# yhw-yhw/TalkSHOW

Hardware: NVIDIA H100
Metric: smplx_motion_frames_per_sec (higher is better)
Workload: dtype f32

## Files before the change

talkshow_b200/csrc/api.cu:

```cuda
#include "convstack.h"
#include "pixelcnn.h"

using namespace ts;

static std::string g_create_err;

float* ts_engine::upload(const std::vector<float>& h) {
  if (host_only) return nullptr;
  void* d = dmalloc(h.size() * sizeof(float));
  TS_CUDA(cudaMemcpy(d, h.data(), h.size() * sizeof(float), cudaMemcpyHostToDevice));
  return (float*)d;
}
unsigned short* ts_engine::upload(const std::vector<unsigned short>& h) {
  if (host_only) return nullptr;
  void* d = dmalloc(h.size() * sizeof(unsigned short));
  TS_CUDA(cudaMemcpy(d, h.data(), h.size() * sizeof(unsigned short), cudaMemcpyHostToDevice));
  return (unsigned short*)d;
}
void* ts_engine::dmalloc(size_t bytes) {
  if (host_only) return nullptr;
  void* d = nullptr;
  TS_CUDA(cudaMalloc(&d, bytes ? bytes : 16));
  (alloc_sink ? *alloc_sink : owned).push_back(d);
  return d;
// ... 208 lines not shown
      TS_CUDA(cudaEventRecord(e->aux_fork, s));
      TS_CUDA(cudaStreamWaitEvent(e->aux_stream, e->aux_fork, 0));
    }
    for (int w = 0; w < 2; ++w) {
      cudaStream_t sw = (w == 1 && par) ? e->aux_stream : s;
      Act3 y = run_vq_decode(e, e->conv->vq[w], idx_c + (size_t)w * B * T, B, T, sw);
      act_to_btc(e, y, e->conv->vq[w].out_dim, poses, c0 + c1, w ? c0 : 0, sw);
    }
    if (par) {
      TS_CUDA(cudaEventRecord(e->aux_join, e->aux_stream));
      TS_CUDA(cudaStreamWaitEvent(s, e->aux_join, 0));
    }
  };
  e->ws.begin_sizing();
  body();
  size_t need = e->ws.need;
  e->ws.buf.ensure(need + 256);
  e->ws.begin(need);
  body();
  TS_API_END(e)
}
```

talkshow_b200/csrc/common.h:

```cpp
#pragma once
#include <cuda_runtime.h>
#include <stdint.h>

#include <cstdarg>
#include <cstdio>
#include <cstring>
#include <map>
#include <stdexcept>
#include <string>
#include <vector>

#include "../../include/talkshow_b200.h"

namespace ts {

struct Error : std::runtime_error {
  int code;
  Error(int c, const std::string& m) : std::runtime_error(m), code(c) {}
};

[[noreturn]] inline void fail(int code, const char* fmt, ...) {
  char buf[1024];
  va_list ap;
  va_start(ap, fmt);
// ... 47 lines not shown
    bytes = n;
  }
  void release() {
    if (p) cudaFree(p);
    p = nullptr;
    bytes = 0;
  }
  template <class T>
  T* as() const { return (T*)p; }
};

struct Workspace {
  DevBuf buf;
  size_t off = 0;
  size_t need = 0;
  bool sizing = false;
  void begin_sizing() { sizing = true; off = 0; need = 0; }
  void begin(size_t) { sizing = false; off = 0; }
  template <class T>
  T* alloc(size_t n) {
    size_t b = (n * sizeof(T) + 255) & ~size_t(255);
    size_t o = off;
    off += b;
    if (off > need) need = off;
    if (sizing) return nullptr;
    if (off > buf.bytes) fail(TS_ERR_CUDA, "workspace overflow (%zu > %zu)", off, buf.bytes);
    return (T*)((char*)buf.p + o);
  }
};

struct Layer {
  float* W = nullptr;
  float* W_hi = nullptr;
// ... 110 lines not shown
```

talkshow_b200/csrc/convstack.cu:

```cuda
#include "convstack.h"

#include <cmath>

namespace ts {

static const double BN_EPS = 1e-5;

struct Folded {
  std::vector<double> a, b;
};

static Folded bn_fold(const Ckpt& ck, const std::string& p, int c) {
  const float* g = ck.f32(p + "weight", {c});
  const float* be = ck.f32(p + "bias", {c});
  const float* mu = ck.f32(p + "running_mean", {c});
  const float* var = ck.f32(p + "running_var", {c});
  Folded f;
  f.a.resize(c);
  f.b.resize(c);
  for (int i = 0; i < c; ++i) {
    double a = (double)g[i] / std::sqrt((double)var[i] + BN_EPS);
    f.a[i] = a;
    f.b[i] = (double)be[i] - (double)mu[i] * a;
  }
// ... 186 lines not shown
  conv_auto(e, v.project, h, 1, 1, 0, y, h.T, ACT_NONE, nullptr, s);
  return y;
}

Act3 run_vq_decode(ts_engine* e, const VQNet& v, const int64_t* idx, int B, int T, cudaStream_t s) {
  Act3 q = new_act(e, B, T, 64, 0, s);
  gather_rows(e, v.codebook, 64, idx, q, s);
  return run_decoder(e, v, q, s);
}

}

using namespace ts;

template <class F>
static void run_sized(ts_engine* e, F&& body) {
  e->ws.begin_sizing();
  body();
  size_t need = e->ws.need;
  e->ws.buf.ensure(need + 256);
  e->ws.begin(need);
  body();
}

extern "C" int ts_latent_rows(int M) {
  int m = (M + 2 - 4) / 2 + 1;
  return (m + 2 - 4) / 2 + 1;
}

extern "C" int ts_load_audioenc(ts_engine* e, const ts_tensor* tensors, int n) {
  TS_API_BEGIN(e)
  Ckpt ck(tensors, n);
  if (!e->conv) e->conv = new ConvStacks();
  LoadScope scope(e, "audioenc");
  Trunk t;
  pack_trunk(e, ck, "", 64, 256, &t);
// ... 10 lines not shown
  if (!e->conv) e->conv = new ConvStacks();
  LoadScope scope(e, which ? "vq1" : "vq0");
  VQNet v;
  pack_vq(e, ck, &v);
  e->conv->vq[which] = v;
  scope.commit();
  TS_API_END(e)
}

extern "C" int ts_audio_encode(ts_engine* e, const float* mfcc, float* out, int B, int M, void* stream) {
  TS_API_BEGIN(e)
  ts::require_device(e);
  if (!e->conv || !e->conv->audio_loaded) fail(TS_ERR_NOT_LOADED, "audio encoder weights not loaded");
  if (B <= 0 || M < 4) fail(TS_ERR_INVALID, "ts_audio_encode: B=%d M=%d", B, M);
  cudaStream_t s = (cudaStream_t)stream;
  run_sized(e, [&] {
    Act3 x = new_act(e, B, M, 64, 1, s);
    nct_to_act(e, mfcc, 64, x, s);
    Act3 y = run_trunk(e, e->conv->audio, x, s);
    act_to_nct(e, y, 256, out, s);
  });
  TS_API_END(e)
}

extern "C" int ts_vq_decode(ts_engine* e, int which, const int64_t* idx, float* out, int B, int T, void* stream) {
  TS_API_BEGIN(e)
  ts::require_device(e);
  if (which < 0 || which > 1 || !e->conv || !e->conv->vq[which].loaded) fail(TS_ERR_NOT_LOADED, "vq[%d] weights not loaded", which);
  if (B <= 0 || T <= 0) fail(TS_ERR_INVALID, "ts_vq_decode: B=%d T=%d", B, T);
  cudaStream_t s = (cudaStream_t)stream;
  const VQNet& v = e->conv->vq[which];
  run_sized(e, [&] {
    Act3 y = run_vq_decode(e, v, idx, B, T, s);
    act_to_nct(e, y, v.out_dim, out, s);
  });
  TS_API_END(e)
}

extern "C" int ts_vq_encode(ts_engine* e, int which, const float* poses, int64_t* idx, float* e_out, int B, int F,
                            void* stream) {
  TS_API_BEGIN(e)
  ts::require_device(e);
  if (which < 0 || which > 1 || !e->conv || !e->conv->vq[which].loaded) fail(TS_ERR_NOT_LOADED, "vq[%d] weights not loaded", which);
  if (B <= 0 || F < 4) fail(TS_ERR_INVALID, "ts_vq_encode: B=%d F=%d", B, F);
  cudaStream_t s = (cudaStream_t)stream;
  const VQNet& v = e->conv->vq[which];
  run_sized(e, [&] {
    Act3 x = new_act(e, B, F, pad4(v.out_dim), 1, s);
    btc_to_act(e, poses, v.out_dim, x, s);
    Act3 h = run_trunk(e, v.enc, x, s);
    Act3 z = new_act(e, B, h.T, 64, 0, s);
    conv1d(e, v.pre_vq, h, 1, 1, 0, z, h.T, ACT_NONE, nullptr, s);
    vq_argmin(e, v.codebook, v.ee, v.ncodes, z, idx, s);
    if (e_out) {
      Act3 q = new_act(e, B, h.T, 64, 0, s);
      gather_rows(e, v.codebook, 64, idx, q, s);
      act_to_nct(e, q, 64, e_out, s);
    }
  });
  TS_API_END(e)
}
```

talkshow_b200/csrc/face.cu:

```cuda
#include <cuda_fp16.h>
#include "convstack.h"

#include <memory>
#include "pixelcnn.h"

namespace ts {

static const int W2V_K[7] = {10, 3, 3, 3, 3, 2, 2};
static const int W2V_S[7] = {5, 2, 2, 2, 2, 2, 2};

struct EncLayer {
  Layer qkv, out, ff1, ff2;
  float *ln1_g, *ln1_b, *ln2_g, *ln2_b;
};

struct FaceNet {
  float* conv0_w = nullptr;
  float *gn_g = nullptr, *gn_b = nullptr;
  Layer conv[7];
  float *fp_ln_g = nullptr, *fp_ln_b = nullptr;
  Layer fproj, posconv;
  unsigned short* pos_w16 = nullptr;
  float pos_unscale = 1.f;
  float *enc_ln_g = nullptr, *enc_ln_b = nullptr;
// ... 1321 lines not shown
  }
  delete e->face;
  e->face = Fp.release();
  scope.commit();
  TS_API_END(e)
}

extern "C" int ts_face_forward(ts_engine* e, const float* wave, const float* id, float* out, int B, int N, int frame, void* stream) {
  TS_API_BEGIN(e)
  ts::require_device(e);
  if (!e->face) fail(TS_ERR_NOT_LOADED, "face weights not loaded");
  if (B <= 0 || N < 400 || frame <= 0) fail(TS_ERR_INVALID, "ts_face_forward: B=%d N=%d frame=%d (need >= 400 samples)", B, N, frame);
  cudaStream_t s = (cudaStream_t)stream;
  e->ws.begin_sizing();
  face_run(e, wave, id, out, B, N, frame, s);
  size_t need = e->ws.need;
  e->ws.buf.ensure(need + 256);
  e->ws.begin(need);
  face_run(e, wave, id, out, B, N, frame, s);
  TS_API_END(e)
}
```

talkshow_b200/csrc/gemm_tc.cu:

```cuda
#include <cuda.h>
#include <cuda_fp16.h>

#include "kernels.h"

namespace ts {

constexpr int TC_BM = 128, TC_BN = 128;
constexpr int TC_BK = 32;
constexpr int TC_STAGES = 3;
constexpr int TC_TILE_BYTES = 128 * 128;
constexpr int TC_STAGE_BYTES = 4 * TC_TILE_BYTES;
constexpr int TC_THREADS = 384;
constexpr int TC_SMEM = TC_STAGES * TC_STAGE_BYTES + 1024  + 256 ;
constexpr int TC_SLD = TC_BN + 4;
static_assert(TC_BM * TC_SLD * 4 + 2 * TC_BM * 8 <= TC_STAGES * TC_STAGE_BYTES, "parked tile must fit in the operand ring");
static_assert(TC_SMEM <= 227 * 1024, "shared memory per block");

struct TcArgs {
  int taps, cblocks, stride;
  int C;
  int rows_in, off, T_out, nbatch;
  int Rs;
  int N;
  float* c_hi;
  float* c_lo;
  long c_bs, c_rs;
  const float* bias;
  const float* r_hi;
  const float* r_lo;
  long r_bs, r_rs;
  int act;
  int chunk;
  float oscale;
  unsigned short* c_h16;
  unsigned short* c_l16;
};

__device__ __forceinline__ uint32_t s_u32(const void* p) { return (uint32_t)__cvta_generic_to_shared(p); }
__device__ __forceinline__ void mb_init(uint64_t* b, int c) { asm volatile("mbarrier.init.shared::cta.b64 [%0], %1;" ::"r"(s_u32(b)), "r"(c)); }
__device__ __forceinline__ void mb_expect(uint64_t* b, uint32_t bytes) {
  asm volatile("mbarrier.arrive.expect_tx.shared::cta.b64 _, [%0], %1;" ::"r"(s_u32(b)), "r"(bytes) : "memory");
}
__device__ __forceinline__ void mb_arrive_lane0(uint64_t* b, int lane) {
  asm volatile("{\n.reg .pred p;\nsetp.eq.s32 p, %1, 0;\n@p mbarrier.arrive.shared::cta.b64 _, [%0];\n}\n" ::"r"(s_u32(b)), "r"(lane) : "memory");
}
__device__ __forceinline__ void mb_wait(uint64_t* b, uint32_t parity) {
  asm volatile(
      "{\n.reg .pred p;\nTCW:\nmbarrier.try_wait.parity.shared::cta.b64 p, [%0], %1;\n@p bra TCD;\nbra TCW;\nTCD:\n}\n" ::"r"(s_u32(b)),
      "r"(parity)
      : "memory");
}
__device__ __forceinline__ void tma_3d(void* dst, const CUtensorMap* m, int c0, int c1, int c2, uint64_t* bar) {
  asm volatile("cp.async.bulk.tensor.3d.shared::cluster.global.tile.mbarrier::complete_tx::bytes [%0], [%1, {%2, %3, %4}], [%5];" ::"r"(s_u32(dst)),
               "l"(m), "r"(c0), "r"(c1), "r"(c2), "r"(s_u32(bar))
               : "memory");
}
__device__ __forceinline__ void tma_2d(void* dst, const CUtensorMap* m, int c0, int c1, uint64_t* bar) {
  asm volatile("cp.async.bulk.tensor.2d.shared::cluster.global.tile.mbarrier::complete_tx::bytes [%0], [%1, {%2, %3}], [%4];" ::"r"(s_u32(dst)),
               "l"(m), "r"(c0), "r"(c1), "r"(s_u32(bar))
               : "memory");
}
__device__ __forceinline__ uint64_t wg_desc(uint32_t smem_addr) {
  uint64_t d = 0;
  d |= (uint64_t)((smem_addr >> 4) & 0x3fff);
  d |= (uint64_t)1 << 16;
  d |= (uint64_t)(1024 >> 4) << 32;
  d |= (uint64_t)1 << 62;
  return d;
}
#define TC_ACC64                                                                                                              \
  "{%0, %1, %2, %3, %4, %5, %6, %7, %8, %9, %10, %11, %12, %13, %14, %15, %16, %17, %18, %19, %20, %21, %22, %23, %24, %25, " \
  "%26, %27, %28, %29, %30, %31, %32, %33, %34, %35, %36, %37, %38, %39, %40, %41, %42, %43, %44, %45, %46, %47, %48, %49, "   \
  "%50, %51, %52, %53, %54, %55, %56, %57, %58, %59, %60, %61, %62, %63}"
#define TC_ACC64_OPS(d)                                                                                                       \
  "+f"(d[0]), "+f"(d[1]), "+f"(d[2]), "+f"(d[3]), "+f"(d[4]), "+f"(d[5]), "+f"(d[6]), "+f"(d[7]), "+f"(d[8]), "+f"(d[9]),     \
      "+f"(d[10]), "+f"(d[11]), "+f"(d[12]), "+f"(d[13]), "+f"(d[14]), "+f"(d[15]), "+f"(d[16]), "+f"(d[17]), "+f"(d[18]),    \
      "+f"(d[19]), "+f"(d[20]), "+f"(d[21]), "+f"(d[22]), "+f"(d[23]), "+f"(d[24]), "+f"(d[25]), "+f"(d[26]), "+f"(d[27]),    \
      "+f"(d[28]), "+f"(d[29]), "+f"(d[30]), "+f"(d[31]), "+f"(d[32]), "+f"(d[33]), "+f"(d[34]), "+f"(d[35]), "+f"(d[36]),    \
      "+f"(d[37]), "+f"(d[38]), "+f"(d[39]), "+f"(d[40]), "+f"(d[41]), "+f"(d[42]), "+f"(d[43]), "+f"(d[44]), "+f"(d[45]),    \
      "+f"(d[46]), "+f"(d[47]), "+f"(d[48]), "+f"(d[49]), "+f"(d[50]), "+f"(d[51]), "+f"(d[52]), "+f"(d[53]), "+f"(d[54]),    \
      "+f"(d[55]), "+f"(d[56]), "+f"(d[57]), "+f"(d[58]), "+f"(d[59]), "+f"(d[60]), "+f"(d[61]), "+f"(d[62]), "+f"(d[63])
template <bool F16>
// ... 12 lines not shown
#undef TC_ACC64
#undef TC_ACC64_OPS
__device__ __forceinline__ void wgmma_fence() { asm volatile("wgmma.fence.sync.aligned;" ::: "memory"); }
__device__ __forceinline__ void wgmma_commit() { asm volatile("wgmma.commit_group.sync.aligned;" ::: "memory"); }
template <int N>
__device__ __forceinline__ void wgmma_wait() { asm volatile("wgmma.wait_group.sync.aligned %0;" ::"n"(N) : "memory"); }

__device__ __forceinline__ float tc_act(float v, int act) {
  if (act == ACT_RELU) return v > 0.f ? v : 0.f;
  if (act == ACT_LRELU) return v > 0.f ? v : 0.2f * v;
  if (act == ACT_GELU) return 0.5f * v * (1.0f + erff(v * 0.70710678118654752440f));
  return v;
}

template <int ACT, int CG, int SLD>
__device__ __forceinline__ void tc_writeout(const TcArgs& P, const float* S, const long* rowc, const long* rowr, int n0) {
  const int et = threadIdx.x - 128;
  const int c4 = (et % CG) * 4, n = n0 + c4;
  if (n >= P.N) return;
  const int nv = min(4, P.N - n);
  float bv[4] = {0.f, 0.f, 0.f, 0.f};
  if (P.bias)
    for (int q = 0; q < nv; ++q) bv[q] = P.bias[n + q];
  const float osc = P.oscale;
  const bool rvec = nv == 4 && P.r_hi && (((P.r_bs | P.r_rs) & 3) == 0) && ((reinterpret_cast<uintptr_t>(P.r_hi) & 15) == 0) &&
                    (!P.r_lo || (reinterpret_cast<uintptr_t>(P.r_lo) & 15) == 0);
#pragma unroll 4
  for (int r = et / CG; r < TC_BM; r += 256 / CG) {
    const long co = rowc[r];
    if (co < 0) continue;
    const float4 sv = *reinterpret_cast<const float4*>(&S[r * SLD + c4]);
    float o[4] = {sv.x * osc + bv[0], sv.y * osc + bv[1], sv.z * osc + bv[2], sv.w * osc + bv[3]};
    if (P.r_hi) {
      const long roff = rowr[r] + n;
      if (rvec) {
        const float4 rh = *reinterpret_cast<const float4*>(P.r_hi + roff);
        if (P.r_lo) {
          const float4 rl = *reinterpret_cast<const float4*>(P.r_lo + roff);
          o[0] += rh.x + rl.x; o[1] += rh.y + rl.y; o[2] += rh.z + rl.z; o[3] += rh.w + rl.w;
        } else {
          o[0] += rh.x; o[1] += rh.y; o[2] += rh.z; o[3] += rh.w;
        }
      } else {
// ... 35 lines not shown
          P.c_lo[coff + q] = o[q] - h;
        } else {
          P.c_hi[coff + q] = o[q];
        }
      }
    }
  }
}

template <bool F16>
__global__ void __launch_bounds__(TC_THREADS, 1)
tc_gemm_kernel(const __grid_constant__ CUtensorMap mA_hi, const __grid_constant__ CUtensorMap mA_lo,
               const __grid_constant__ CUtensorMap mB_hi, const __grid_constant__ CUtensorMap mB_lo, TcArgs P) {
  extern __shared__ unsigned char tc_smem_raw[];
  unsigned char* smem = reinterpret_cast<unsigned char*>((reinterpret_cast<uintptr_t>(tc_smem_raw) + 1023) & ~uintptr_t(1023));
  uint64_t* full = reinterpret_cast<uint64_t*>(smem + TC_STAGES * TC_STAGE_BYTES);
  uint64_t* empty = full + TC_STAGES;
  const int warp = threadIdx.x >> 5, lane = threadIdx.x & 31;
  const int j0 = blockIdx.y * TC_BM, n0 = blockIdx.x * TC_BN;
  const int nk = P.taps * P.cblocks;
  constexpr int BK = F16 ? 2 * TC_BK : TC_BK;

  if (threadIdx.x == 0) {
    for (int i = 0; i < TC_STAGES; ++i) { mb_init(&full[i], 1); mb_init(&empty[i], 8); }
    asm volatile("fence.mbarrier_init.release.cluster;" ::: "memory");
    asm volatile("prefetch.tensormap [%0];" ::"l"(&mA_hi) : "memory");
    asm volatile("prefetch.tensormap [%0];" ::"l"(&mA_lo) : "memory");
    asm volatile("prefetch.tensormap [%0];" ::"l"(&mB_hi) : "memory");
    asm volatile("prefetch.tensormap [%0];" ::"l"(&mB_lo) : "memory");
  }
  __syncthreads();

  if (warp < 4) {
    if (threadIdx.x == 0) {
      for (int kb = 0; kb < nk; ++kb) {
        const int st = kb % TC_STAGES, ph = (kb / TC_STAGES) & 1;
        mb_wait(&empty[st], ph ^ 1);
        const int tap = kb / P.cblocks, cb = kb - tap * P.cblocks;
        unsigned char* base = smem + st * TC_STAGE_BYTES;
        mb_expect(&full[st], TC_STAGE_BYTES);
        const int c0 = cb * BK, c1 = tap % P.stride, c2 = j0 + tap / P.stride;
        const int kcol = tap * P.C + cb * BK;
        tma_3d(base, &mA_hi, c0, c1, c2, &full[st]);
        tma_3d(base + TC_TILE_BYTES, &mA_lo, c0, c1, c2, &full[st]);
        tma_2d(base + 2 * TC_TILE_BYTES, &mB_hi, kcol, n0, &full[st]);
        tma_2d(base + 3 * TC_TILE_BYTES, &mB_lo, kcol, n0, &full[st]);
      }
    }
    return;
  }

  const int wg = (warp >> 2) - 1;
  float acc[64], sum[64];
#pragma unroll
  for (int i = 0; i < 64; ++i) sum[i] = 0.f;
  for (int c0 = 0; c0 < nk; c0 += P.chunk) {
    const int cend = min(nk, c0 + P.chunk);
    for (int kb = c0; kb < cend; ++kb) {
      const int st = kb % TC_STAGES, ph = (kb / TC_STAGES) & 1;
      mb_wait(&full[st], ph);
      const uint32_t a_hi = s_u32(smem + st * TC_STAGE_BYTES) + wg * 64 * 128, a_lo = a_hi + TC_TILE_BYTES;
      const uint32_t b_hi = s_u32(smem + st * TC_STAGE_BYTES) + 2 * TC_TILE_BYTES, b_lo = b_hi + TC_TILE_BYTES;
      wgmma_fence();
#pragma unroll
      for (int k = 0; k < 4; ++k) {
        const uint32_t o = k * 32;
        wgmma_64x128<F16>(acc, wg_desc(a_lo + o), wg_desc(b_hi + o), (kb > c0) | k);
        wgmma_64x128<F16>(acc, wg_desc(a_hi + o), wg_desc(b_lo + o), 1);
        wgmma_64x128<F16>(acc, wg_desc(a_hi + o), wg_desc(b_hi + o), 1);
      }
      wgmma_commit();
      wgmma_wait<1>();
      __syncwarp();
      if (kb > c0) mb_arrive_lane0(&empty[(kb + TC_STAGES - 1) % TC_STAGES], lane);
    }
    wgmma_wait<0>();
    __syncwarp();
    mb_arrive_lane0(&empty[(cend - 1) % TC_STAGES], lane);
#pragma unroll
    for (int i = 0; i < 64; ++i) sum[i] += acc[i];
  }

  asm volatile("bar.sync 1, 256;" ::: "memory");
  float* S = reinterpret_cast<float*>(smem);
  long* rowc = reinterpret_cast<long*>(S + TC_BM * TC_SLD);
  long* rowr = rowc + TC_BM;
  {
    const int r0 = wg * 64 + (warp & 3) * 16 + (lane >> 2), c0 = 2 * (lane & 3);
#pragma unroll
    for (int i = 0; i < 64; i += 2) {
      const int r = r0 + 8 * ((i >> 1) & 1), c = c0 + 8 * (i >> 2);
      *reinterpret_cast<float2*>(&S[r * TC_SLD + c]) = make_float2(sum[i], sum[i + 1]);
    }
  }
  const int et = threadIdx.x - 128;
  if (et < TC_BM) {
    const int j = j0 + et;
    long co = -1, ro = 0;
    if (j < P.Rs) {
      const long in_row = (long)j * P.stride;
      const int bb = (int)(in_row / P.rows_in);
      const int tin = (int)(in_row - (long)bb * P.rows_in) - P.off;
      if (bb < P.nbatch && tin >= 0 && (tin % P.stride) == 0 && tin / P.stride < P.T_out) {
        const int t = tin / P.stride;
        co = (long)bb * P.c_bs + (long)t * P.c_rs;
        ro = (long)bb * P.r_bs + (long)t * P.r_rs;
      }
    }
    rowc[et] = co;
    rowr[et] = ro;
  }
  asm volatile("bar.sync 1, 256;" ::: "memory");
  if (P.act == ACT_NONE) tc_writeout<ACT_NONE, TC_BN / 4, TC_SLD>(P, S, rowc, rowr, n0);
  else if (P.act == ACT_GELU) tc_writeout<ACT_GELU, TC_BN / 4, TC_SLD>(P, S, rowc, rowr, n0);
  else tc_writeout<-1, TC_BN / 4, TC_SLD>(P, S, rowc, rowr, n0);
}

__global__ void split_kernel(const float* __restrict__ x, float* __restrict__ hi, float* __restrict__ lo, long n) {
  for (long i = blockIdx.x * (long)blockDim.x + threadIdx.x; i < n; i += (long)gridDim.x * blockDim.x) {
    float v = x[i];
    float h = __uint_as_float(__float_as_uint(v) & 0xffffe000u);
    hi[i] = h;
    lo[i] = v - h;
  }
}
void split_hi_lo(ts_engine* e, const float* x, float* hi, float* lo, long n, cudaStream_t s) {
  if (e->ws.sizing || n <= 0) return;
  split_kernel<<<(int)std::min<long>((n + 255) / 256, (long)e->sm_count * 16), 256, 0, s>>>(x, hi, lo, n);
  e->launches++;
  TS_CUDA(cudaGetLastError());
// ... 43 lines not shown
  static EncodeTiledFn fn = nullptr;
  if (!fn) {
    void* p = nullptr;
    cudaDriverEntryPointQueryResult q;
    TS_CUDA(cudaGetDriverEntryPoint("cuTensorMapEncodeTiled", &p, cudaEnableDefault, &q));
    if (!p || q != cudaDriverEntryPointSuccess) fail(TS_ERR_CUDA, "cuTensorMapEncodeTiled entry point unavailable");
    fn = (EncodeTiledFn)p;
  }
  return fn;
}
static CUtensorMap make_map(const void* base, int rank, const cuuint64_t* dims, const cuuint64_t* strides_bytes, const cuuint32_t* box,
                            bool f16 = false) {
  CUtensorMap m;
  cuuint32_t estr[3] = {1, 1, 1};
  CUresult r = get_encode()(&m, f16 ? CU_TENSOR_MAP_DATA_TYPE_FLOAT16 : CU_TENSOR_MAP_DATA_TYPE_FLOAT32, rank, (void*)base, dims, strides_bytes, box, estr, CU_TENSOR_MAP_INTERLEAVE_NONE,
                            CU_TENSOR_MAP_SWIZZLE_128B, CU_TENSOR_MAP_L2_PROMOTION_L2_256B, CU_TENSOR_MAP_FLOAT_OOB_FILL_NONE);
  if (r != CUDA_SUCCESS) fail(TS_ERR_CUDA, "cuTensorMapEncodeTiled failed (%d) rank %d dims %llu,%llu", (int)r, rank, (unsigned long long)dims[0],
                              (unsigned long long)dims[1]);
  return m;
}

bool tc_conv_supported(ts_engine* e, const Layer& L, const Act3& x, int stride, int pd) {
  if (e->tc_f16) {
    if (!L.W_h16 || !x.h16 || x.C % (2 * TC_BK)) return false;
  } else {
    if (!L.W_hi || !x.lo || x.C % TC_BK) return false;
  }
  const int rows_in = x.T + 2 * x.pad + x.tail;
  if (rows_in % stride || (x.pad - pd) % stride || x.pad < pd) return false;
  return true;
}

void tc_conv1d(ts_engine* e, const Layer& L, const Act3& x, int k, int stride, int pd, const Act3& y, int T_out, int act, const Act3* res,
               cudaStream_t s, int y_tmul, int y_toff, int coff) {
  if (e->ws.sizing) return;
  if (!tc_conv_supported(e, L, x, stride, pd)) fail(TS_ERR_INVALID, "tc_conv1d: unsupported geometry");
  if (!y.p && !y.h16) fail(TS_ERR_INVALID, "tc_conv1d: output without storage");
  const bool f16 = e->tc_f16;
  const int esz = f16 ? 2 : 4, bk = f16 ? 2 * TC_BK : TC_BK;
  if (L.taps != k || L.cin != x.C) fail(TS_ERR_INVALID, "tc_conv1d: layer/input mismatch");
  const int rows_in = x.T + 2 * x.pad + x.tail;
  const long R = (long)x.B * rows_in;
  const long Rs = R / stride;
  const void* base_hi = f16 ? (const void*)x.h16 : (const void*)x.p;
  const void* base_lo = f16 ? (const void*)x.l16 : (const void*)x.lo;
  cuuint64_t adims[3] = {(cuuint64_t)x.C, (cuuint64_t)stride, (cuuint64_t)Rs};
  cuuint64_t astr[2] = {(cuuint64_t)x.C * esz, (cuuint64_t)x.C * esz * stride};
  const int tiles_n = (L.N + TC_BN - 1) / TC_BN, tiles_m = (int)((Rs + TC_BM - 1) / TC_BM);
  cuuint32_t abox[3] = {(cuuint32_t)bk, 1, (cuuint32_t)TC_BM};
  CUtensorMap mAh = make_map(base_hi, 3, adims, astr, abox, f16), mAl = make_map(base_lo, 3, adims, astr, abox, f16);
  cuuint64_t bdims[2] = {(cuuint64_t)L.K, (cuuint64_t)L.N};
  cuuint64_t bstr[1] = {(cuuint64_t)L.K * esz};
  cuuint32_t bbox[2] = {(cuuint32_t)bk, (cuuint32_t)TC_BN};
  const void* wh = f16 ? (const void*)L.W_h16 : (const void*)L.W_hi;
// ... 1 lines not shown
  CUtensorMap mBh = make_map(wh, 2, bdims, bstr, bbox, f16), mBl = make_map(wl, 2, bdims, bstr, bbox, f16);
  TcArgs P;
  P.chunk = 256 / bk;
  P.oscale = f16 ? L.w_unscale : 1.f;
  P.c_h16 = y.h16 ? y.row_h16(0, y_toff) + coff : nullptr;
  P.c_l16 = y.h16 ? y.row_l16(0, y_toff) + coff : nullptr;
  P.taps = k; P.cblocks = x.C / bk; P.stride = stride; P.C = x.C;
  P.rows_in = rows_in; P.off = x.pad - pd; P.T_out = T_out; P.nbatch = x.B; P.Rs = (int)Rs; P.N = L.N;
  P.c_hi = y.p ? y.row(0, y_toff) + coff : nullptr; P.c_lo = y.lo ? y.row_lo(0, y_toff) + coff : nullptr;
  P.c_bs = y.bstride(); P.c_rs = (long)y_tmul * y.C;
  P.bias = L.bias;
  P.r_hi = res ? res->row(0, 0) : nullptr;
  P.r_lo = (res && res->lo) ? res->row_lo(0, 0) : nullptr;
  P.r_bs = res ? res->bstride() : 0; P.r_rs = res ? res->C : 0;
  P.act = act;
  if (!e->tc_attr_set) {
    TS_CUDA(cudaFuncSetAttribute(tc_gemm_kernel<false>, cudaFuncAttributeMaxDynamicSharedMemorySize, TC_SMEM));
    TS_CUDA(cudaFuncSetAttribute(tc_gemm_kernel<true>, cudaFuncAttributeMaxDynamicSharedMemorySize, TC_SMEM));
    e->tc_attr_set = true;
  }
  const dim3 grid((unsigned)tiles_n, (unsigned)tiles_m);
  if (f16) tc_gemm_kernel<true><<<grid, TC_THREADS, TC_SMEM, s>>>(mAh, mAl, mBh, mBl, P);
  else tc_gemm_kernel<false><<<grid, TC_THREADS, TC_SMEM, s>>>(mAh, mAl, mBh, mBl, P);
  e->launches++;
  TS_CUDA(cudaGetLastError());
}

void upload_weights(ts_engine* e, const std::vector<float>& W, Layer* L) {
  L->W = e->upload(W);
  std::vector<float> hi, lo;
  split_host(W, &hi, &lo);
  L->W_hi = e->upload(hi);
  L->W_lo = e->upload(lo);
  std::vector<unsigned short> h16, l16;
  L->w_unscale = split16_host(W, &h16, &l16);
  L->W_h16 = e->upload(h16);
// ... 7 lines not shown
}

}

using namespace ts;

extern "C" int ts_set_tensor_cores(ts_engine* e, int enable) {
  if (!e) return TS_ERR_INVALID;
  if (enable < 0 || enable > 6 || enable == 2 || enable == 5) {
    e->err = "ts_set_tensor_cores: modes are 0 (FFMA), 1 / 3 / 4 (3xTF32 wgmma) and 6 (fp16-split wgmma)";
    return TS_ERR_UNSUPPORTED;
  }
  e->use_tc = enable != 0;
  e->tc_f16 = enable == 6;
  return TS_OK;
}

extern "C" int ts_debug_gemm(ts_engine* e, int mode, const float* A, const float* W, const float* bias, float* C, int M, int N, int K, int act,
                             void* stream) {
  TS_API_BEGIN(e)
  cudaStream_t s = (cudaStream_t)stream;
  if (mode == 0) {
    GemmP p;
    p.A = A; p.W = W; p.bias = bias; p.C = C; p.M = M; p.N = N; p.K = K; p.mper = M; p.a_rs = K; p.kc = K; p.a_ts = K; p.c_rs = N; p.act = act; p.ldw = K;
    e->ws.sizing = false;
    launch_gemm(e, p, s);
  } else if (mode == 3) {
    if (K % (2 * TC_BK)) fail(TS_ERR_INVALID, "ts_debug_gemm: K must be a multiple of 64 for the fp16-split path");
    const bool f0 = e->tc_f16;
    e->tc_f16 = true;
    e->ws.sizing = false;
    unsigned short *ah, *al, *wh, *wl;
    TS_CUDA(cudaMalloc(&ah, (size_t)M * K * 2)); TS_CUDA(cudaMalloc(&al, (size_t)M * K * 2));
    TS_CUDA(cudaMalloc(&wh, (size_t)N * K * 2)); TS_CUDA(cudaMalloc(&wl, (size_t)N * K * 2));
    split16_kernel<<<e->sm_count * 8, 256, 0, s>>>(A, ah, al, (long)M * K, 1.f);
    split16_kernel<<<e->sm_count * 8, 256, 0, s>>>(W, wh, wl, (long)N * K, 256.f);
    Layer L;
    L.N = N; L.K = K; L.taps = 1; L.cin = K; L.W_h16 = wh; L.W_l16 = wl; L.w_unscale = 1.f / 256.f; L.bias = const_cast<float*>(bias);
    Act3 x; x.p = const_cast<float*>(A); x.h16 = ah; x.l16 = al; x.split = true; x.B = 1; x.T = M; x.C = K; x.pad = 0;
    Act3 y; y.p = C; y.B = 1; y.T = M; y.C = N; y.pad = 0;
    tc_conv1d(e, L, x, 1, 1, 0, y, M, act, nullptr, s, 1, 0, 0);
    e->tc_f16 = f0;
    TS_CUDA(cudaStreamSynchronize(s));
    cudaFree(ah); cudaFree(al); cudaFree(wh); cudaFree(wl);
  } else if (mode == 1) {
    if (K % TC_BK) fail(TS_ERR_INVALID, "ts_debug_gemm: K must be a multiple of 32 for the tensor-core path");
    const bool f0 = e->tc_f16;
    e->tc_f16 = false;
    e->ws.sizing = false;
    float *ah, *al, *wh, *wl;
    TS_CUDA(cudaMalloc(&ah, (size_t)M * K * 4)); TS_CUDA(cudaMalloc(&al, (size_t)M * K * 4));
    TS_CUDA(cudaMalloc(&wh, (size_t)N * K * 4)); TS_CUDA(cudaMalloc(&wl, (size_t)N * K * 4));
    split_hi_lo(e, A, ah, al, (long)M * K, s);
    split_hi_lo(e, W, wh, wl, (long)N * K, s);
    Layer L;
    L.N = N; L.K = K; L.taps = 1; L.cin = K; L.W_hi = wh; L.W_lo = wl; L.bias = const_cast<float*>(bias);
    Act3 x; x.p = ah; x.lo = al; x.split = true; x.B = 1; x.T = M; x.C = K; x.pad = 0;
    Act3 y; y.p = C; y.B = 1; y.T = M; y.C = N; y.pad = 0;
    tc_conv1d(e, L, x, 1, 1, 0, y, M, act, nullptr, s, 1, 0, 0);
    e->tc_f16 = f0;
    TS_CUDA(cudaStreamSynchronize(s));
    cudaFree(ah); cudaFree(al); cudaFree(wh); cudaFree(wl);
  } else {
    fail(TS_ERR_INVALID, "ts_debug_gemm: mode %d (0 = FFMA, 1 = 3xTF32, 3 = fp16-split)", mode);
  }
  TS_API_END(e)
}
```

talkshow_b200/csrc/lbs.cu:

```cuda
#include "pixelcnn.h"

#include <cmath>
#include <memory>

namespace ts {

constexpr int LBS_J = 55;
constexpr int LBS_NB = 300, LBS_NE = 100, LBS_NP = 486;
constexpr int LBS_KC = 588;
constexpr int LBS_MAXF = 4096;

struct SmplxModel {
  int V = 0, nextra = 0, nlmk = 0;
  Layer dirs;
  Layer beta_dirs;
  float* v_template = nullptr;
  float* J0 = nullptr;
  float* JS = nullptr;
  float* wT = nullptr;
  float* pose_mean = nullptr;
  int* parents = nullptr;
  int* extra_idx = nullptr;
  int* lmk_tri = nullptr;
  float* lmk_bary = nullptr;
// ... 289 lines not shown
      e->launches++;
      GemmP g;
      g.A = coef; g.W = M->dirs.W; g.bias = vbase; g.C = vposed;
      g.M = nf; g.N = N3; g.K = LBS_KC; g.mper = nf; g.a_bs = 0; g.a_rs = LBS_KC; g.kc = LBS_KC; g.a_ts = LBS_KC;
      g.c_bs = 0; g.c_rs = N3; g.ldw = LBS_KC;
      launch_gemm(e, g, s);
      lbs_skin_kernel<<<dim3(cdiv(V, 256), nf), 256, 0, s>>>(vposed, A, M->wT, vout, V, nf);
      e->launches++;
      lbs_extra_kernel<<<nf, 256, 0, s>>>(vout, M->extra_idx, M->lmk_tri, M->lmk_bary, jout, V, M->nextra, M->nlmk, NJ);
      e->launches++;
      TS_CUDA(cudaGetLastError());
    }
  };
  e->ws.begin_sizing();
  body();
  const size_t need = e->ws.need;
  e->ws.buf.ensure(need + 256);
  e->ws.begin(need);
  body();
  TS_API_END(e)
}
```

talkshow_b200/csrc/mfcc.cu:

```cuda
#include <cmath>

#include "convstack.h"

namespace ts {

constexpr int MF_NFFT = 2048, MF_NFREQ = 1025, MF_NFREQ_PAD = 1028, MF_NMEL = 256, MF_NMFCC = 64, MF_SR = 22000;
constexpr int MF_HOP = 734;

struct MfccTables {
  Layer dft, mel, dct;
  float* window = nullptr;
  int rs_orig = 0, rs_new = 0, rs_width = 0, rs_kw = 0;
  float* rs_kernel = nullptr;
};


static Layer make_layer(ts_engine* e, const std::vector<float>& W, int N, int K) {
  Layer L;
  L.N = N; L.K = K; L.taps = 1; L.cin = K;
  L.W = e->upload(W);
  return L;
}

static MfccTables* tables(ts_engine* e) {
// ... 185 lines not shown

using namespace ts;

extern "C" int ts_mfcc_frames(int N, int sr) { return (N > 0 && sr > 0) ? mfcc_frames(N, sr) : 0; }

extern "C" int ts_mfcc(ts_engine* e, const float* wave, float* out, int B, int N, int sr, void* stream) {
  TS_API_BEGIN(e)
  if (e->host_only) fail(TS_ERR_UNSUPPORTED, "host-only engine cannot execute");
  if (B <= 0 || N < MF_NFFT || sr <= 0) fail(TS_ERR_INVALID, "ts_mfcc: B=%d N=%d sr=%d (need >= %d samples)", B, N, sr, MF_NFFT);
  cudaStream_t s = (cudaStream_t)stream;
  auto body = [&] {
    Act3 m = run_mfcc(e, wave, B, N, sr, 0, s);
    act_to_nct(e, m, MF_NMFCC, out, s);
  };
  e->ws.begin_sizing(); body();
  size_t need = e->ws.need;
  e->ws.buf.ensure(need + 256);
  e->ws.begin(need); body();
  TS_API_END(e)
}
```

talkshow_b200/csrc/pixelcnn.cu:

```cuda
#include "pixelcnn.h"
#include "convstack.h"

#include <algorithm>
#include <memory>
#include <cmath>

namespace ts {


struct Job {
  int epi, layer, col, nrows, K, ncol;
  bool pairs;
  int rofs = 0;
};

constexpr double PIX_ROWCOST = 0.0;

static int rows_cap(int K) { return std::min(PIX_MAXROWS, (PIX_WBUF / (K + 1)) & ~3); }

static void push_vert0(std::vector<std::vector<Job>>& st, int D, bool split) {
  if (split) {
    st.push_back({{EPI_VERT0, 0, 0, 2 * D, 6 * D, 1, true}});
    st.push_back({{EPI_VERT0, 0, 1, 2 * D, 6 * D, 1, true}});
  } else {
// ... 1321 lines not shown
}

extern "C" int ts_pixelcnn_generate(ts_engine* e, const float* aud, const int64_t* label, const float* noise,
                                    int64_t* idx_out, float* logits_out, int B, int T, const int64_t* pre_latents, int T0,
                                    void* stream) {
  TS_API_BEGIN(e)
  check_pix(e, B, T);
  if (T0 < 0 || (T0 > 0 && !pre_latents)) fail(TS_ERR_INVALID, "pixelcnn: T0=%d without pre_latents", T0);
  cudaStream_t s = (cudaStream_t)stream;
  auto body = [&] {
    Act3 a = new_act(e, B, T0 + T, 256, 0, s);
    nct_to_act(e, aud, 256, a, s);
    pixelcnn_generate_act(e, a, label, noise, idx_out, logits_out, B, T, pre_latents, T0, s);
  };
  e->ws.begin_sizing(); body();
  size_t need = e->ws.need;
  e->ws.buf.ensure(need + 256);
  e->ws.begin(need); body();
  TS_API_END(e)
}

extern "C" int ts_pixelcnn_logits(ts_engine* e, const float* aud, const int64_t* label, const int64_t* codes,
                                  float* logits_out, int B, int T, void* stream) {
  TS_API_BEGIN(e)
  check_pix(e, B, T);
  cudaStream_t s = (cudaStream_t)stream;
  auto body = [&] {
    Act3 a = new_act(e, B, T, 256, 0, s);
    nct_to_act(e, aud, 256, a, s);
    float* steps = e->ws.alloc<float>((size_t)2 * T * B * PIX_NCODE);
    int64_t* dummy = e->ws.alloc<int64_t>(16);
    pixelcnn_generate_act(e, a, label, nullptr, dummy, steps, B, 0, codes, T, s, true);
    if (!e->ws.sizing) {
      long n = (long)2 * T * B * PIX_NCODE;
      logits_to_ref_kernel<<<(int)std::min<long>((n + 255) / 256, (long)e->sm_count * 16), 256, 0, s>>>(steps, logits_out, B, T);
      e->launches++;
      TS_CUDA(cudaGetLastError());
    }
  };
  e->ws.begin_sizing(); body();
  size_t need = e->ws.need;
  e->ws.buf.ensure(need + 256);
  e->ws.begin(need); body();
  TS_API_END(e)
}
```

Baseline: 193,600.

## Make TC GEMM persistent with atomic tile scheduler and dedicated epilogue warpgroup

Converts the warp-specialized wgmma GEMM into a persistent kernel. CTAs pull tiles from a global atomic counter (zeroed per call from a workspace counter slot), and a separate 128-thread epilogue warpgroup writes out the parked accumulator tile while the math warpgroups start the next tile. It also halves the K-row per stage to 64 bytes with 64B swizzle, uses more stages, and rebalances registers with setmaxnreg. The aim is to hide epilogue and launch tail costs. The price is an extra memset per call, more barrier bookkeeping, and risk of descriptor or swizzle mismatch.

```diff
diff --git a/talkshow_b200/csrc/api.cu b/talkshow_b200/csrc/api.cu
--- a/talkshow_b200/csrc/api.cu
+++ b/talkshow_b200/csrc/api.cu
@@ -246,9 +246,7 @@
   };
   e->ws.begin_sizing();
   body();
-  size_t need = e->ws.need;
-  e->ws.buf.ensure(need + 256);
-  e->ws.begin(need);
+  e->ws.begin(s);
   body();
   TS_API_END(e)
 }
diff --git a/talkshow_b200/csrc/common.h b/talkshow_b200/csrc/common.h
--- a/talkshow_b200/csrc/common.h
+++ b/talkshow_b200/csrc/common.h
@@ -85,9 +85,23 @@
   DevBuf buf;
   size_t off = 0;
   size_t need = 0;
+  int* ctr = nullptr;
+  int nctr = 0, ctr_need = 0;
   bool sizing = false;
-  void begin_sizing() { sizing = true; off = 0; need = 0; }
-  void begin(size_t) { sizing = false; off = 0; }
+  void begin_sizing() { sizing = true; off = 0; need = 0; ctr_need = 0; }
+  void begin(cudaStream_t s) {
+    buf.ensure(need + 256 + (size_t)ctr_need * sizeof(int));
+    sizing = false;
+    off = 0;
+    nctr = 0;
+    ctr = (int*)((char*)buf.p + need);
+    if (ctr_need) TS_CUDA(cudaMemsetAsync(ctr, 0, (size_t)ctr_need * sizeof(int), s));
+  }
+  int* counter() {
+    if (sizing) { ++ctr_need; return nullptr; }
+    if (nctr >= ctr_need) fail(TS_ERR_CUDA, "workspace: more GEMM launches (%d) than the sizing pass counted", nctr + 1);
+    return ctr + nctr++;
+  }
   template <class T>
   T* alloc(size_t n) {
     size_t b = (n * sizeof(T) + 255) & ~size_t(255);
diff --git a/talkshow_b200/csrc/convstack.cu b/talkshow_b200/csrc/convstack.cu
--- a/talkshow_b200/csrc/convstack.cu
+++ b/talkshow_b200/csrc/convstack.cu
@@ -224,12 +224,10 @@
 using namespace ts;
 
 template <class F>
-static void run_sized(ts_engine* e, F&& body) {
+static void run_sized(ts_engine* e, cudaStream_t s, F&& body) {
   e->ws.begin_sizing();
   body();
-  size_t need = e->ws.need;
-  e->ws.buf.ensure(need + 256);
-  e->ws.begin(need);
+  e->ws.begin(s);
   body();
 }
 
@@ -270,7 +268,7 @@
   if (!e->conv || !e->conv->audio_loaded) fail(TS_ERR_NOT_LOADED, "audio encoder weights not loaded");
   if (B <= 0 || M < 4) fail(TS_ERR_INVALID, "ts_audio_encode: B=%d M=%d", B, M);
   cudaStream_t s = (cudaStream_t)stream;
-  run_sized(e, [&] {
+  run_sized(e, s, [&] {
     Act3 x = new_act(e, B, M, 64, 1, s);
     nct_to_act(e, mfcc, 64, x, s);
     Act3 y = run_trunk(e, e->conv->audio, x, s);
@@ -286,7 +284,7 @@
   if (B <= 0 || T <= 0) fail(TS_ERR_INVALID, "ts_vq_decode: B=%d T=%d", B, T);
   cudaStream_t s = (cudaStream_t)stream;
   const VQNet& v = e->conv->vq[which];
-  run_sized(e, [&] {
+  run_sized(e, s, [&] {
     Act3 y = run_vq_decode(e, v, idx, B, T, s);
     act_to_nct(e, y, v.out_dim, out, s);
   });
@@ -301,7 +299,7 @@
   if (B <= 0 || F < 4) fail(TS_ERR_INVALID, "ts_vq_encode: B=%d F=%d", B, F);
   cudaStream_t s = (cudaStream_t)stream;
   const VQNet& v = e->conv->vq[which];
-  run_sized(e, [&] {
+  run_sized(e, s, [&] {
     Act3 x = new_act(e, B, F, pad4(v.out_dim), 1, s);
     btc_to_act(e, poses, v.out_dim, x, s);
     Act3 h = run_trunk(e, v.enc, x, s);
diff --git a/talkshow_b200/csrc/face.cu b/talkshow_b200/csrc/face.cu
--- a/talkshow_b200/csrc/face.cu
+++ b/talkshow_b200/csrc/face.cu
@@ -1359,9 +1359,7 @@
   cudaStream_t s = (cudaStream_t)stream;
   e->ws.begin_sizing();
   face_run(e, wave, id, out, B, N, frame, s);
-  size_t need = e->ws.need;
-  e->ws.buf.ensure(need + 256);
-  e->ws.begin(need);
+  e->ws.begin(s);
   face_run(e, wave, id, out, B, N, frame, s);
   TS_API_END(e)
 }
diff --git a/talkshow_b200/csrc/gemm_tc.cu b/talkshow_b200/csrc/gemm_tc.cu
--- a/talkshow_b200/csrc/gemm_tc.cu
+++ b/talkshow_b200/csrc/gemm_tc.cu
@@ -7,13 +7,16 @@
 
 constexpr int TC_BM = 128, TC_BN = 128;
 constexpr int TC_BK = 32;
-constexpr int TC_STAGES = 3;
-constexpr int TC_TILE_BYTES = 128 * 128;
+constexpr int TC_KROW = 64;
+constexpr int TC_TILE_BYTES = 128 * TC_KROW;
 constexpr int TC_STAGE_BYTES = 4 * TC_TILE_BYTES;
-constexpr int TC_THREADS = 384;
-constexpr int TC_SMEM = TC_STAGES * TC_STAGE_BYTES + 1024  + 256 ;
+constexpr int TC_STAGES = 128 * 1024 / TC_STAGE_BYTES;
+constexpr int TC_THREADS = 512;
+constexpr int TC_EPI_THREADS = 128;
+constexpr int TC_RING = 4;
 constexpr int TC_SLD = TC_BN + 4;
-static_assert(TC_BM * TC_SLD * 4 + 2 * TC_BM * 8 <= TC_STAGES * TC_STAGE_BYTES, "parked tile must fit in the operand ring");
+constexpr int TC_PARK_BYTES = TC_BM * TC_SLD * 4;
+constexpr int TC_SMEM = TC_STAGES * TC_STAGE_BYTES + TC_PARK_BYTES + 2 * TC_BM * 8  + 256  + 1024 ;
 static_assert(TC_SMEM <= 227 * 1024, "shared memory per block");
 
 struct TcArgs {
@@ -34,6 +37,8 @@
   float oscale;
   unsigned short* c_h16;
   unsigned short* c_l16;
+  int tiles, tiles_n;
+  int* counter;
 };
 
 __device__ __forceinline__ uint32_t s_u32(const void* p) { return (uint32_t)__cvta_generic_to_shared(p); }
@@ -60,12 +65,13 @@
                "l"(m), "r"(c0), "r"(c1), "r"(s_u32(bar))
                : "memory");
 }
+__device__ __forceinline__ void mb_arrive(uint64_t* b) { asm volatile("mbarrier.arrive.shared::cta.b64 _, [%0];" ::"r"(s_u32(b)) : "memory"); }
 __device__ __forceinline__ uint64_t wg_desc(uint32_t smem_addr) {
   uint64_t d = 0;
   d |= (uint64_t)((smem_addr >> 4) & 0x3fff);
   d |= (uint64_t)1 << 16;
-  d |= (uint64_t)(1024 >> 4) << 32;
-  d |= (uint64_t)1 << 62;
+  d |= (uint64_t)(8 * TC_KROW >> 4) << 32;
+  d |= (uint64_t)(TC_KROW == 128 ? 1 : 2) << 62;
   return d;
 }
 #define TC_ACC64                                                                                                              \
@@ -108,8 +114,7 @@
 }
 
 template <int ACT, int CG, int SLD>
-__device__ __forceinline__ void tc_writeout(const TcArgs& P, const float* S, const long* rowc, const long* rowr, int n0) {
-  const int et = threadIdx.x - 128;
+__device__ __forceinline__ void tc_writeout(const TcArgs& P, const float* S, const long* rowc, const long* rowr, int n0, int et) {
   const int c4 = (et % CG) * 4, n = n0 + c4;
   if (n >= P.N) return;
   const int nv = min(4, P.N - n);
@@ -120,7 +125,7 @@
   const bool rvec = nv == 4 && P.r_hi && (((P.r_bs | P.r_rs) & 3) == 0) && ((reinterpret_cast<uintptr_t>(P.r_hi) & 15) == 0) &&
                     (!P.r_lo || (reinterpret_cast<uintptr_t>(P.r_lo) & 15) == 0);
 #pragma unroll 4
-  for (int r = et / CG; r < TC_BM; r += 256 / CG) {
+  for (int r = et / CG; r < TC_BM; r += TC_EPI_THREADS / CG) {
     const long co = rowc[r];
     if (co < 0) continue;
     const float4 sv = *reinterpret_cast<const float4*>(&S[r * SLD + c4]);
@@ -186,15 +191,25 @@
                const __grid_constant__ CUtensorMap mB_hi, const __grid_constant__ CUtensorMap mB_lo, TcArgs P) {
   extern __shared__ unsigned char tc_smem_raw[];
   unsigned char* smem = reinterpret_cast<unsigned char*>((reinterpret_cast<uintptr_t>(tc_smem_raw) + 1023) & ~uintptr_t(1023));
-  uint64_t* full = reinterpret_cast<uint64_t*>(smem + TC_STAGES * TC_STAGE_BYTES);
+  float* S = reinterpret_cast<float*>(smem + TC_STAGES * TC_STAGE_BYTES);
+  long* rowc = reinterpret_cast<long*>(smem + TC_STAGES * TC_STAGE_BYTES + TC_PARK_BYTES);
+  long* rowr = rowc + TC_BM;
+  uint64_t* full = reinterpret_cast<uint64_t*>(rowr + TC_BM);
   uint64_t* empty = full + TC_STAGES;
+  uint64_t* tfull = empty + TC_STAGES;
+  uint64_t* tempty = tfull + TC_RING;
+  uint64_t* pfull = tempty + TC_RING;
+  uint64_t* pempty = pfull + 1;
+  volatile int* ring = reinterpret_cast<volatile int*>(pempty + 1);
   const int warp = threadIdx.x >> 5, lane = threadIdx.x & 31;
-  const int j0 = blockIdx.y * TC_BM, n0 = blockIdx.x * TC_BN;
   const int nk = P.taps * P.cblocks;
-  constexpr int BK = F16 ? 2 * TC_BK : TC_BK;
+  constexpr int BK = TC_KROW / (F16 ? 2 : 4);
 
   if (threadIdx.x == 0) {
     for (int i = 0; i < TC_STAGES; ++i) { mb_init(&full[i], 1); mb_init(&empty[i], 8); }
+    for (int i = 0; i < TC_RING; ++i) { mb_init(&tfull[i], 1); mb_init(&tempty[i], 256 + TC_EPI_THREADS); }
+    mb_init(pfull, 256);
+    mb_init(pempty, TC_EPI_THREADS);
     asm volatile("fence.mbarrier_init.release.cluster;" ::: "memory");
     asm volatile("prefetch.tensormap [%0];" ::"l"(&mA_hi) : "memory");
     asm volatile("prefetch.tensormap [%0];" ::"l"(&mA_lo) : "memory");
@@ -204,9 +219,19 @@
   __syncthreads();
 
   if (warp < 4) {
-    if (threadIdx.x == 0) {
-      for (int kb = 0; kb < nk; ++kb) {
-        const int st = kb % TC_STAGES, ph = (kb / TC_STAGES) & 1;
+    asm volatile("setmaxnreg.dec.sync.aligned.u32 40;");
+    if (threadIdx.x != 0) return;
+    int g = 0;
+    for (int it = 0;; ++it) {
+      const int slot = it % TC_RING;
+      mb_wait(&tempty[slot], ((it / TC_RING) & 1) ^ 1);
+      const int t = atomicAdd(P.counter, 1);
+      ring[slot] = t;
+      mb_arrive(&tfull[slot]);
+      if (t >= P.tiles) return;
+      const int j0 = (t / P.tiles_n) * TC_BM, n0 = (t % P.tiles_n) * TC_BN;
+      for (int kb = 0; kb < nk; ++kb, ++g) {
+        const int st = g % TC_STAGES, ph = (g / TC_STAGES) & 1;
         mb_wait(&empty[st], ph ^ 1);
         const int tap = kb / P.cblocks, cb = kb - tap * P.cblocks;
         unsigned char* base = smem + st * TC_STAGE_BYTES;
@@ -219,73 +244,92 @@
         tma_2d(base + 3 * TC_TILE_BYTES, &mB_lo, kcol, n0, &full[st]);
       }
     }
-    return;
-  }
-
-  const int wg = (warp >> 2) - 1;
-  float acc[64], sum[64];
+  }
+
+  if (warp < 12) {
+    asm volatile("setmaxnreg.inc.sync.aligned.u32 168;");
+    const int wg = (warp >> 2) - 1;
+    int g = 0;
+    for (int it = 0;; ++it) {
+      const int slot = it % TC_RING;
+      mb_wait(&tfull[slot], (it / TC_RING) & 1);
+      const int t = ring[slot];
+      mb_arrive(&tempty[slot]);
+      if (t >= P.tiles) return;
+      float acc[64], sum[64];
 #pragma unroll
-  for (int i = 0; i < 64; ++i) sum[i] = 0.f;
-  for (int c0 = 0; c0 < nk; c0 += P.chunk) {
-    const int cend = min(nk, c0 + P.chunk);
-    for (int kb = c0; kb < cend; ++kb) {
-      const int st = kb % TC_STAGES, ph = (kb / TC_STAGES) & 1;
-      mb_wait(&full[st], ph);
-      const uint32_t a_hi = s_u32(smem + st * TC_STAGE_BYTES) + wg * 64 * 128, a_lo = a_hi + TC_TILE_BYTES;
-      const uint32_t b_hi = s_u32(smem + st * TC_STAGE_BYTES) + 2 * TC_TILE_BYTES, b_lo = b_hi + TC_TILE_BYTES;
-      wgmma_fence();
+      for (int i = 0; i < 64; ++i) sum[i] = 0.f;
+      for (int c0 = 0; c0 < nk; c0 += P.chunk) {
+        const int cend = min(nk, c0 + P.chunk);
+        for (int kb = c0; kb < cend; ++kb) {
+          const int gk = g + kb, st = gk % TC_STAGES, ph = (gk / TC_STAGES) & 1;
+          mb_wait(&full[st], ph);
+          const uint32_t a_hi = s_u32(smem + st * TC_STAGE_BYTES) + wg * 64 * TC_KROW, a_lo = a_hi + TC_TILE_BYTES;
+          const uint32_t b_hi = s_u32(smem + st * TC_STAGE_BYTES) + 2 * TC_TILE_BYTES, b_lo = b_hi + TC_TILE_BYTES;
+          wgmma_fence();
 #pragma unroll
-      for (int k = 0; k < 4; ++k) {
-        const uint32_t o = k * 32;
-        wgmma_64x128<F16>(acc, wg_desc(a_lo + o), wg_desc(b_hi + o), (kb > c0) | k);
-        wgmma_64x128<F16>(acc, wg_desc(a_hi + o), wg_desc(b_lo + o), 1);
-        wgmma_64x128<F16>(acc, wg_desc(a_hi + o), wg_desc(b_hi + o), 1);
-      }
-      wgmma_commit();
-      wgmma_wait<1>();
-      __syncwarp();
-      if (kb > c0) mb_arrive_lane0(&empty[(kb + TC_STAGES - 1) % TC_STAGES], lane);
+          for (int k = 0; k < TC_KROW / 32; ++k) {
+            const uint32_t o = k * 32;
+            wgmma_64x128<F16>(acc, wg_desc(a_lo + o), wg_desc(b_hi + o), (kb > c0) | k);
+            wgmma_64x128<F16>(acc, wg_desc(a_hi + o), wg_desc(b_lo + o), 1);
+            wgmma_64x128<F16>(acc, wg_desc(a_hi + o), wg_desc(b_hi + o), 1);
+          }
+          wgmma_commit();
+          wgmma_wait<1>();
+          __syncwarp();
+          if (kb > c0) mb_arrive_lane0(&empty[(gk + TC_STAGES - 1) % TC_STAGES], lane);
+        }
+        wgmma_wait<0>();
+        __syncwarp();
+        mb_arrive_lane0(&empty[(g + cend - 1) % TC_STAGES], lane);
+#pragma unroll
+        for (int i = 0; i < 64; ++i) sum[i] += acc[i];
+      }
+      g += nk;
+      mb_wait(pempty, (it & 1) ^ 1);
+      const int r0 = wg * 64 + (warp & 3) * 16 + (lane >> 2), cl = 2 * (lane & 3);
+#pragma unroll
+      for (int i = 0; i < 64; i += 2) {
+        const int r = r0 + 8 * ((i >> 1) & 1), c = cl + 8 * (i >> 2);
+        *reinterpret_cast<float2*>(&S[r * TC_SLD + c]) = make_float2(sum[i], sum[i + 1]);
+      }
+      mb_arrive(pfull);
     }
-    wgmma_wait<0>();
-    __syncwarp();
-    mb_arrive_lane0(&empty[(cend - 1) % TC_STAGES], lane);
-#pragma unroll
-    for (int i = 0; i < 64; ++i) sum[i] += acc[i];
-  }
-
-  asm volatile("bar.sync 1, 256;" ::: "memory");
-  float* S = reinterpret_cast<float*>(smem);
-  long* rowc = reinterpret_cast<long*>(S + TC_BM * TC_SLD);
-  long* rowr = rowc + TC_BM;
-  {
-    const int r0 = wg * 64 + (warp & 3) * 16 + (lane >> 2), c0 = 2 * (lane & 3);
-#pragma unroll
-    for (int i = 0; i < 64; i += 2) {
-      const int r = r0 + 8 * ((i >> 1) & 1), c = c0 + 8 * (i >> 2);
-      *reinterpret_cast<float2*>(&S[r * TC_SLD + c]) = make_float2(sum[i], sum[i + 1]);
+  }
+
+  asm volatile("setmaxnreg.dec.sync.aligned.u32 96;");
+  const int et = threadIdx.x - 384;
+  for (int it = 0;; ++it) {
+    const int slot = it % TC_RING;
+    mb_wait(&tfull[slot], (it / TC_RING) & 1);
+    const int t = ring[slot];
+    mb_arrive(&tempty[slot]);
+    if (t >= P.tiles) return;
+    const int j0 = (t / P.tiles_n) * TC_BM, n0 = (t % P.tiles_n) * TC_BN;
+    asm volatile("bar.sync 1, 128;" ::: "memory");
+    {
+      const int j = j0 + et;
+      long co = -1, ro = 0;
+      if (j < P.Rs) {
+        const long in_row = (long)j * P.stride;
+        const int bb = (int)(in_row / P.rows_in);
+        const int tin = (int)(in_row - (long)bb * P.rows_in) - P.off;
+        if (bb < P.nbatch && tin >= 0 && (tin % P.stride) == 0 && tin / P.stride < P.T_out) {
+          const int tt = tin / P.stride;
+          co = (long)bb * P.c_bs + (long)tt * P.c_rs;
+          ro = (long)bb * P.r_bs + (long)tt * P.r_rs;
+        }
+      }
+      rowc[et] = co;
+      rowr[et] = ro;
     }
-  }
-  const int et = threadIdx.x - 128;
-  if (et < TC_BM) {
-    const int j = j0 + et;
-    long co = -1, ro = 0;
-    if (j < P.Rs) {
-      const long in_row = (long)j * P.stride;
-      const int bb = (int)(in_row / P.rows_in);
-      const int tin = (int)(in_row - (long)bb * P.rows_in) - P.off;
-      if (bb < P.nbatch && tin >= 0 && (tin % P.stride) == 0 && tin / P.stride < P.T_out) {
-        const int t = tin / P.stride;
-        co = (long)bb * P.c_bs + (long)t * P.c_rs;
-        ro = (long)bb * P.r_bs + (long)t * P.r_rs;
-      }
-    }
-    rowc[et] = co;
-    rowr[et] = ro;
-  }
-  asm volatile("bar.sync 1, 256;" ::: "memory");
-  if (P.act == ACT_NONE) tc_writeout<ACT_NONE, TC_BN / 4, TC_SLD>(P, S, rowc, rowr, n0);
-  else if (P.act == ACT_GELU) tc_writeout<ACT_GELU, TC_BN / 4, TC_SLD>(P, S, rowc, rowr, n0);
-  else tc_writeout<-1, TC_BN / 4, TC_SLD>(P, S, rowc, rowr, n0);
+    asm volatile("bar.sync 1, 128;" ::: "memory");
+    mb_wait(pfull, it & 1);
+    if (P.act == ACT_NONE) tc_writeout<ACT_NONE, TC_BN / 4, TC_SLD>(P, S, rowc, rowr, n0, et);
+    else if (P.act == ACT_GELU) tc_writeout<ACT_GELU, TC_BN / 4, TC_SLD>(P, S, rowc, rowr, n0, et);
+    else tc_writeout<-1, TC_BN / 4, TC_SLD>(P, S, rowc, rowr, n0, et);
+    mb_arrive(pempty);
+  }
 }
 
 __global__ void split_kernel(const float* __restrict__ x, float* __restrict__ hi, float* __restrict__ lo, long n) {
@@ -359,17 +403,18 @@
   CUtensorMap m;
   cuuint32_t estr[3] = {1, 1, 1};
   CUresult r = get_encode()(&m, f16 ? CU_TENSOR_MAP_DATA_TYPE_FLOAT16 : CU_TENSOR_MAP_DATA_TYPE_FLOAT32, rank, (void*)base, dims, strides_bytes, box, estr, CU_TENSOR_MAP_INTERLEAVE_NONE,
-                            CU_TENSOR_MAP_SWIZZLE_128B, CU_TENSOR_MAP_L2_PROMOTION_L2_256B, CU_TENSOR_MAP_FLOAT_OOB_FILL_NONE);
+                            TC_KROW == 128 ? CU_TENSOR_MAP_SWIZZLE_128B : CU_TENSOR_MAP_SWIZZLE_64B, CU_TENSOR_MAP_L2_PROMOTION_L2_256B, CU_TENSOR_MAP_FLOAT_OOB_FILL_NONE);
   if (r != CUDA_SUCCESS) fail(TS_ERR_CUDA, "cuTensorMapEncodeTiled failed (%d) rank %d dims %llu,%llu", (int)r, rank, (unsigned long long)dims[0],
                               (unsigned long long)dims[1]);
   return m;
 }
 
 bool tc_conv_supported(ts_engine* e, const Layer& L, const Act3& x, int stride, int pd) {
+  const bool planned = e->ws.sizing && x.split;
   if (e->tc_f16) {
-    if (!L.W_h16 || !x.h16 || x.C % (2 * TC_BK)) return false;
+    if (!L.W_h16 || !(x.h16 || planned) || x.C % (2 * TC_BK)) return false;
   } else {
-    if (!L.W_hi || !x.lo || x.C % TC_BK) return false;
+    if (!L.W_hi || !(x.lo || planned) || x.C % TC_BK) return false;
   }
   const int rows_in = x.T + 2 * x.pad + x.tail;
   if (rows_in % stride || (x.pad - pd) % stride || x.pad < pd) return false;
@@ -378,11 +423,12 @@
 
 void tc_conv1d(ts_engine* e, const Layer& L, const Act3& x, int k, int stride, int pd, const Act3& y, int T_out, int act, const Act3* res,
                cudaStream_t s, int y_tmul, int y_toff, int coff) {
+  int* counter = e->ws.counter();
   if (e->ws.sizing) return;
   if (!tc_conv_supported(e, L, x, stride, pd)) fail(TS_ERR_INVALID, "tc_conv1d: unsupported geometry");
   if (!y.p && !y.h16) fail(TS_ERR_INVALID, "tc_conv1d: output without storage");
   const bool f16 = e->tc_f16;
-  const int esz = f16 ? 2 : 4, bk = f16 ? 2 * TC_BK : TC_BK;
+  const int esz = f16 ? 2 : 4, bk = TC_KROW / esz;
   if (L.taps != k || L.cin != x.C) fail(TS_ERR_INVALID, "tc_conv1d: layer/input mismatch");
   const int rows_in = x.T + 2 * x.pad + x.tail;
   const long R = (long)x.B * rows_in;
@@ -414,12 +460,14 @@
   P.r_lo = (res && res->lo) ? res->row_lo(0, 0) : nullptr;
   P.r_bs = res ? res->bstride() : 0; P.r_rs = res ? res->C : 0;
   P.act = act;
+  P.tiles = tiles_n * tiles_m; P.tiles_n = tiles_n;
+  P.counter = counter;
   if (!e->tc_attr_set) {
     TS_CUDA(cudaFuncSetAttribute(tc_gemm_kernel<false>, cudaFuncAttributeMaxDynamicSharedMemorySize, TC_SMEM));
     TS_CUDA(cudaFuncSetAttribute(tc_gemm_kernel<true>, cudaFuncAttributeMaxDynamicSharedMemorySize, TC_SMEM));
     e->tc_attr_set = true;
   }
-  const dim3 grid((unsigned)tiles_n, (unsigned)tiles_m);
+  const int grid = std::min(P.tiles, e->sm_count);
   if (f16) tc_gemm_kernel<true><<<grid, TC_THREADS, TC_SMEM, s>>>(mAh, mAl, mBh, mBl, P);
   else tc_gemm_kernel<false><<<grid, TC_THREADS, TC_SMEM, s>>>(mAh, mAl, mBh, mBl, P);
   e->launches++;
@@ -457,6 +505,13 @@
   e->use_tc = enable != 0;
   e->tc_f16 = enable == 6;
   return TS_OK;
+}
+
+static void debug_tc_gemm(ts_engine* e, const Layer& L, const Act3& x, const Act3& y, int M, int act, cudaStream_t s) {
+  e->ws.begin_sizing();
+  tc_conv1d(e, L, x, 1, 1, 0, y, M, act, nullptr, s, 1, 0, 0);
+  e->ws.begin(s);
+  tc_conv1d(e, L, x, 1, 1, 0, y, M, act, nullptr, s, 1, 0, 0);
 }
 
 extern "C" int ts_debug_gemm(ts_engine* e, int mode, const float* A, const float* W, const float* bias, float* C, int M, int N, int K, int act,
@@ -482,7 +537,7 @@
     L.N = N; L.K = K; L.taps = 1; L.cin = K; L.W_h16 = wh; L.W_l16 = wl; L.w_unscale = 1.f / 256.f; L.bias = const_cast<float*>(bias);
     Act3 x; x.p = const_cast<float*>(A); x.h16 = ah; x.l16 = al; x.split = true; x.B = 1; x.T = M; x.C = K; x.pad = 0;
     Act3 y; y.p = C; y.B = 1; y.T = M; y.C = N; y.pad = 0;
-    tc_conv1d(e, L, x, 1, 1, 0, y, M, act, nullptr, s, 1, 0, 0);
+    debug_tc_gemm(e, L, x, y, M, act, s);
     e->tc_f16 = f0;
     TS_CUDA(cudaStreamSynchronize(s));
     cudaFree(ah); cudaFree(al); cudaFree(wh); cudaFree(wl);
@@ -500,7 +555,7 @@
     L.N = N; L.K = K; L.taps = 1; L.cin = K; L.W_hi = wh; L.W_lo = wl; L.bias = const_cast<float*>(bias);
     Act3 x; x.p = ah; x.lo = al; x.split = true; x.B = 1; x.T = M; x.C = K; x.pad = 0;
     Act3 y; y.p = C; y.B = 1; y.T = M; y.C = N; y.pad = 0;
-    tc_conv1d(e, L, x, 1, 1, 0, y, M, act, nullptr, s, 1, 0, 0);
+    debug_tc_gemm(e, L, x, y, M, act, s);
     e->tc_f16 = f0;
     TS_CUDA(cudaStreamSynchronize(s));
     cudaFree(ah); cudaFree(al); cudaFree(wh); cudaFree(wl);
diff --git a/talkshow_b200/csrc/lbs.cu b/talkshow_b200/csrc/lbs.cu
--- a/talkshow_b200/csrc/lbs.cu
+++ b/talkshow_b200/csrc/lbs.cu
@@ -327,9 +327,7 @@
   };
   e->ws.begin_sizing();
   body();
-  const size_t need = e->ws.need;
-  e->ws.buf.ensure(need + 256);
-  e->ws.begin(need);
+  e->ws.begin(s);
   body();
   TS_API_END(e)
 }
diff --git a/talkshow_b200/csrc/mfcc.cu b/talkshow_b200/csrc/mfcc.cu
--- a/talkshow_b200/csrc/mfcc.cu
+++ b/talkshow_b200/csrc/mfcc.cu
@@ -223,8 +223,6 @@
     act_to_nct(e, m, MF_NMFCC, out, s);
   };
   e->ws.begin_sizing(); body();
-  size_t need = e->ws.need;
-  e->ws.buf.ensure(need + 256);
-  e->ws.begin(need); body();
+  e->ws.begin(s); body();
   TS_API_END(e)
 }
diff --git a/talkshow_b200/csrc/pixelcnn.cu b/talkshow_b200/csrc/pixelcnn.cu
--- a/talkshow_b200/csrc/pixelcnn.cu
+++ b/talkshow_b200/csrc/pixelcnn.cu
@@ -1359,9 +1359,7 @@
     pixelcnn_generate_act(e, a, label, noise, idx_out, logits_out, B, T, pre_latents, T0, s);
   };
   e->ws.begin_sizing(); body();
-  size_t need = e->ws.need;
-  e->ws.buf.ensure(need + 256);
-  e->ws.begin(need); body();
+  e->ws.begin(s); body();
   TS_API_END(e)
 }
 
@@ -1384,8 +1382,6 @@
     }
   };
   e->ws.begin_sizing(); body();
-  size_t need = e->ws.need;
-  e->ws.buf.ensure(need + 256);
-  e->ws.begin(need); body();
+  e->ws.begin(s); body();
   TS_API_END(e)
 }
```

Result: no change. 192,700 (median of 6 runs) (-0.4%).
